# linomp/INF560-approximate-pattern-matching

Measured on AMD Instinct MI355X. Metric: window-DP-cells/sec, higher is better.
Workload: dtype u32

## Files before the change

inf560-approximate-pattern-matching_amd/csrc/apm_scan.hip:

```cpp
#include "apm_state.h"
#include "apm_core.h"

#include <algorithm>
#include <cstdlib>
#include <cstring>

__global__ void apm_popcount_kernel(const uint32_t *w, unsigned long long n, unsigned long long *sum) {
    unsigned long long acc = 0;
    for (unsigned long long i = (unsigned long long)blockIdx.x * blockDim.x + threadIdx.x; i < n; i += (unsigned long long)gridDim.x * blockDim.x)
        acc += (unsigned long long)__popc(w[i]);
    for (int d = 32; d; d >>= 1) acc += __shfl_down(acc, d, 64);
    if ((threadIdx.x & 63) == 0 && acc) atomicAdd(sum, acc);
}

__global__ void apm_popcount_listed_kernel(const uint32_t *w, const uint32_t *blist, const uint32_t *n_listed, const uint32_t *clist_cnt, int regions, unsigned long long *sum) {
    unsigned long long acc = 0;
    const unsigned long long n = (unsigned long long)*n_listed * 64ull, t0 = (unsigned long long)blockIdx.x * blockDim.x + threadIdx.x;
    for (unsigned long long i = t0; i < n; i += (unsigned long long)gridDim.x * blockDim.x)
        acc += (unsigned long long)__popc(w[(unsigned long long)blist[i >> 6] * 64ull + (i & 63ull)]);
    for (unsigned long long i = t0; i < (unsigned long long)regions; i += (unsigned long long)gridDim.x * blockDim.x) acc += clist_cnt[i];
    for (int d = 32; d; d >>= 1) acc += __shfl_down(acc, d, 64);
    if ((threadIdx.x & 63) == 0 && acc) atomicAdd(sum, acc);
}

// ... 163 lines not shown
    va.o_prefix = V.o_prefix;
    va.o_r2s = V.o_r2s;
    va.o_slots = V.o_slots;
    va.o_kext = V.o_kext;
    va.o_pat = V.o_pat;
    va.o_masks = V.o_masks;
    va.o_kinfo = V.o_kinfo;
    va.o_pinfo = V.o_pinfo;
    va.o_rc = V.o_rc;
    va.kinfo = D.d_kinfo;
    va.pinfo = reinterpret_cast<const uint2 *>(D.d_pinfo);
    va.kpart = D.d_kpart;
    va.pats = D.d_descs;
    va.n_pats = (int)V.descs.size();
    va.nk = (int)V.kinfo.size();
    va.band = g.band;
    va.code_shift = S.code_shift;
    va.stride = S.stride;
    return va;
}

static int run_fused(apm_ctx *ctx, DeviceState &ds, const ShardGeom &g, const SieveRange &r, ShortTails &tails, bool *ran) {
    const SievePlan &S = ctx->plan.sieve;
    bool fused_ok = scan_env().fused < 0 ? S.stride == 8 : scan_env().fused != 0;
    std::vector<ApmFusedArgs> fargs;
    std::vector<size_t> fa_index;
    for (size_t v = 0; fused_ok && v < S.launches.size(); ++v) {
        const VerifyLaunch &V = S.launches[v];
        DevVerify &D = ds.verify[v];
        ApmFusedArgs fa{};
        fa.s = sieve_args(S, g, r, ds.d_sieve_bmp);
        fa.v = verify_args(ctx, V, D, g, std::min<int64_t>(g.je, g.nrel - V.m_min + 1));
#ifdef APM_MEASURE
        if (!ds.d_stats) HIP_TRY(ctx, hipMalloc((void **)&ds.d_stats, APM_STATS_BYTES));
        fa.v.stats = ds.d_stats;
#endif
        if (!D.fused_threads) {
            D.fused_blocks_per_cu = apm_fused_geometry(fa, &D.fused_threads);
            if (D.fused_blocks_per_cu < 1) D.fused_threads = -1;
        }
        if (D.fused_threads < 64) fused_ok = false;
        if (fa.v.je > g.jb) { fargs.push_back(fa); fa_index.push_back(v); }
    }
    if (!fused_ok) return APM_OK;
    for (ApmFusedArgs &fa : fargs) {
        tails.ride_with(fa.s);
        const DevVerify &D = ds.verify[fa_index[&fa - fargs.data()]];
#ifdef APM_MEASURE
        HIP_TRY(ctx, hipMemsetAsync(ds.d_stats, 0, APM_STATS_BYTES, ds.stream));
#endif
        fa.v.work = ds.d_work;
        APM_LAUNCH(ctx, ds, "fused", APM_PICK(g, apm_launch_fused)(fa, D.fused_threads, ds.n_cu * D.fused_blocks_per_cu, &ds.work_epoch, ds.stream));
    }
    *ran = true;
    return APM_OK;
}

static int sieve_pass(apm_ctx *ctx, DeviceState &ds, const ShardGeom &g, SieveRange &r, ShortTails &tails, int v) {
    const SievePlan &S = ctx->plan.sieve;
    ApmSieve2Args sv = sieve_args(S, g, r, v < 0 ? ds.d_sieve_bmp : ds.verify[(size_t)v].d_bmp18);
    sv.masks = ds.d_masks;
    if (v >= 0) {
        const VerifyLaunch &V = S.launches[(size_t)v];
        const DevVerify &D = ds.verify[(size_t)v];
        sv.cf_image = reinterpret_cast<const uint4 *>(D.d_cf);
        sv.cf_len = (int)V.cf_image.size();
        sv.cf_o_rrec = V.cf_o_rrec;
// ... 1 lines not shown
        sv.cf_threads = D.cf_threads;
        sv.cf_blocks_per_cu = D.cf_blocks_per_cu;
        sv.cf_o_dp = V.cf_o_dp;
        sv.cf_dp_k = ctx->k;
        sv.cf_dp_cols = V.cf_dp_cols;
    }
    if (v < 0 || tails.n <= 512) tails.ride_with(sv);
    const bool use_blist = scan_env().blist && sv.cf_image != nullptr;
    r.blist_ctr = nullptr;
    if (use_blist) {
        sv.blist = ds.d_blist;
        sv.blist_ctr = APM_BLIST_CTR(ds.d_work, ds.sieve_epoch & 1);
        sv.blist_ctr_next = APM_BLIST_CTR(ds.d_work, (ds.sieve_epoch + 1) & 1);
        r.blist_ctr = sv.blist_ctr;
    }
    r.clist_regions = 0;
    if (use_blist && scan_env().clist) {
        const size_t want = (size_t)r.n_mask_blocks * (size_t)kClistPerBlock + (size_t)kClistMaxRegions * 64;
        const int grc = grow_device_buffer(ctx, ds, (void **)&ds.d_clist, &ds.clist_cap, want, 4);
        if (grc) return grc;
        if (!ds.d_clist_cnt) HIP_TRY(ctx, hipMalloc((void **)&ds.d_clist_cnt, (size_t)kClistMaxRegions * 4));
        const int regions = apm_sieve2cf_blocks(sv, ds.n_cu);
        if (regions >= 1 && regions <= kClistMaxRegions) {
            r.clist_regions = regions;
            r.clist_region_cap = scan_env().clist_region_cap ? (uint32_t)scan_env().clist_region_cap
                                                             : (uint32_t)std::max<int64_t>(64, r.n_mask_blocks * kClistPerBlock / regions);
            sv.clist = ds.d_clist;
            sv.clist_cnt = ds.d_clist_cnt;
            sv.clist_cap = r.clist_region_cap;
        }
    }
    ds.last_clist_regions = r.clist_regions;
    ds.last_blist_ctr = r.blist_ctr;
    HIP_TRY(ctx, APM_PICK(g, apm_launch_sieve2)(sv, ds.n_cu, ds.stream, scan_env().cf_dp_diag != 0, &ds.last_sieve_waves, &ds.last_cf_dp_form));
    if (use_blist) ++ds.sieve_epoch;
    return note_launch(ctx, ds, "sieve");
}

static int verify_pass(apm_ctx *ctx, DeviceState &ds, const ShardGeom &g, const SieveRange &r, size_t v, int64_t je_v) {
    DevVerify &D = ds.verify[v];
    ApmVerifyArgs va = verify_args(ctx, ctx->plan.sieve.launches[v], D, g, je_v);
    va.masks = ds.d_masks;
    if (r.blist_ctr) {
        va.blist = ds.d_blist;
        va.blist_ctr = r.blist_ctr;
    }
    if (r.clist_regions) {
        va.clist = ds.d_clist;
        va.clist_cnt = ds.d_clist_cnt;
        va.clist_cap = r.clist_region_cap;
        va.clist_regions = r.clist_regions;
        va.clist_min_batch = scan_env().clist_min_batch;
    }
    va.tile0 = r.p_lo;
    va.n_mask_blocks = r.n_mask_blocks;
#ifdef APM_MEASURE
    if (!ds.d_stats) HIP_TRY(ctx, hipMalloc((void **)&ds.d_stats, APM_STATS_BYTES));
    HIP_TRY(ctx, hipMemsetAsync(ds.d_stats, 0, APM_STATS_BYTES, ds.stream));
    va.stats = ds.d_stats;
#endif
    va.work = ds.d_work;
    if (!D.blocks_per_cu) D.blocks_per_cu = apm_verify_geometry(va, &D.threads);
    APM_LAUNCH(ctx, ds, "verify", APM_PICK(g, apm_launch_verify)(va, D.threads, ds.n_cu * D.blocks_per_cu, &ds.work_epoch, ds.stream));
    return APM_OK;
}

static int run_sieve_verify(apm_ctx *ctx, DeviceState &ds, const ShardGeom &g, SieveRange &r, ShortTails &tails) {
    const SievePlan &S = ctx->plan.sieve;
    r.n_mask_blocks = (r.nchunks() + 3) / 4;
    int rc = grow_device_buffer(ctx, ds, (void **)&ds.d_masks, &ds.masks_cap, (size_t)r.n_mask_blocks * 64 + 64, 4);
    if (rc) return rc;
    rc = grow_device_buffer(ctx, ds, (void **)&ds.d_blist, &ds.blist_cap, (size_t)r.n_mask_blocks + 64, 4);
    if (rc) return rc;
    ds.last_mask_blocks = r.n_mask_blocks;
    bool per_launch = S.per_launch_sieve;
    for (size_t v = 0; per_launch && v < S.launches.size(); ++v) {
        const VerifyLaunch &V = S.launches[v];
        DevVerify &D = ds.verify[v];
        if (!D.cf_threads) {
            D.cf_blocks_per_cu = apm_sieve2cf_geometry((int)V.cf_image.size(), apm_cf_dp_form(V.cf_o_dp > 0, ctx->k, scan_env().cf_dp_diag != 0), &D.cf_threads);
            if (D.cf_blocks_per_cu < 1) D.cf_threads = -1;
        }
        if (D.cf_threads < 64) per_launch = false;
    }
    bool any_pass = false;
    for (size_t v = 0; v < S.launches.size(); ++v) {
        const int64_t je_v = std::min<int64_t>(g.je, g.nrel - S.launches[v].m_min + 1);
        if (je_v <= g.jb) continue;
        if (per_launch || !any_pass) {
            rc = sieve_pass(ctx, ds, g, r, tails, per_launch ? (int)v : -1);
// ... 243 lines not shown
int scan_shard(apm_ctx *ctx, DeviceState &ds, const ShardText &sh, uint64_t own_begin, uint64_t own_end, unsigned long long *d_counts,
               const ApmPosSink *rec) {
    const uint8_t *d_text = sh.text;
    uint64_t text_off = sh.text_off, text_len = sh.text_len;
    const uint64_t n_total = sh.n_total;
    const bool sieve_on = ctx->plan.sieve.on;
    const uint64_t lim32 = (uint64_t)APM_SIEVE_MAX_BYTES - 4096;
    const uint64_t mis = (uint64_t)(reinterpret_cast<uintptr_t>(d_text) & 15u);
    if (sieve_on && mis != 0 && text_off >= mis && text_len > 0) {
        d_text -= mis;
        text_off -= mis;
        text_len += mis;
    }
    if (!sieve_on || text_len < lim32 || (reinterpret_cast<uintptr_t>(d_text) & 15u) != 0 || own_begin < text_off)
        return scan_shard_one(ctx, ds, ShardText{d_text, text_off, text_len, n_total}, own_begin, own_end, d_counts, rec);
    const uint64_t k = (uint64_t)ctx->k;
    const uint64_t oe = std::min(own_end, n_total > k ? n_total - k : 0);
    const uint64_t m_max = (uint64_t)std::max(ctx->plan.m_max, 1), step = (uint64_t)3 << 30;
    for (uint64_t b = own_begin; b < oe;) {
        const uint64_t e = std::min(oe, b + step);
        const uint64_t sb = text_off + ((b - text_off) & ~(uint64_t)15);
        const uint64_t se = std::min(text_off + text_len, e + m_max + 31);
        const int rc = scan_shard_one(ctx, ds, ShardText{d_text + (sb - text_off), sb, se - sb, n_total}, b, e, d_counts, rec);
        if (rc) return rc;
        b = e;
    }
    return APM_OK;
}

int sieve_candidates(apm_ctx *ctx, DeviceState &ds, double *value) {
    *value = 0;
    if (!ds.d_masks || ds.last_mask_blocks <= 0) return APM_OK;
    HIP_TRY(ctx, hipSetDevice(ds.dev));
    if (!ds.d_stats) HIP_TRY(ctx, hipMalloc((void **)&ds.d_stats, APM_STATS_BYTES));
    unsigned long long *d_sum = ds.d_stats + 7;
    HIP_TRY(ctx, hipMemsetAsync(d_sum, 0, 8, ds.stream));
    if (ds.last_clist_regions)
        hipLaunchKernelGGL(apm_popcount_listed_kernel, dim3(1024), dim3(256), 0, ds.stream, ds.d_masks, ds.d_blist, ds.last_blist_ctr, ds.d_clist_cnt, ds.last_clist_regions, d_sum);
    else
        hipLaunchKernelGGL(apm_popcount_kernel, dim3(1024), dim3(256), 0, ds.stream, ds.d_masks, (unsigned long long)ds.last_mask_blocks * 64ull, d_sum);
    unsigned long long h = 0;
    HIP_TRY(ctx, hipMemcpyAsync(&h, d_sum, 8, hipMemcpyDeviceToHost, ds.stream));
    HIP_TRY(ctx, hipStreamSynchronize(ds.stream));
    *value = (double)h;
    return APM_OK;
}
```

inf560-approximate-pattern-matching_amd/csrc/apm_sieve.h:

```cpp
#ifndef APM_SIEVE_H
#define APM_SIEVE_H

#include "apm_internal.h"

struct ApmSieve2Args {
    const uint8_t *text;
    int64_t avail_pad;
    int64_t tile0;
    int64_t nchunks;
    const uint4 *bitmap;
    int code_shift;
    int stride;
    uint32_t *masks;
    uint32_t *blist;
    uint32_t *blist_ctr, *blist_ctr_next;
    uint32_t *clist;
    uint32_t *clist_cnt;
    uint32_t clist_cap;
    int n_main_blocks;
    int n_tail;
    ApmTailArgs tail;
    const uint4 *cf_image;
    int cf_len, cf_o_rrec, cf_o_lrec;
    int cf_o_dp, cf_dp_k, cf_dp_cols;
    int cf_threads, cf_blocks_per_cu;
#ifdef APM_MEASURE
    int skip_mask;
#endif
};
#define APM_SIEVE_MAX_BYTES (((int64_t)1 << 32) - ((int64_t)64 << 20))
#define APM_CF_WAVE_BYTES 1552
#define APM_CF_DP_PEND_BYTES 128
#define APM_CF_DP_COLS 30
#define APM_CF_DP_SLOTS 7
static inline int apm_cf_dp_form(bool dp, int k, bool diag_on) { return !dp ? 0 : (diag_on && k <= 3 ? 2 : 1); }
const void *apm_sieve2cfdg_fn();
int apm_sieve2cf_geometry(int cf_len, int dp_form, int *threads);
int apm_sieve2cf_blocks(const ApmSieve2Args &a, int n_cu);

struct ApmVerifyArgs {
    const uint8_t *text;
    int64_t avail;
    int64_t avail_pad;
    int64_t jb, je, nrel;
    const uint4 *image;
    int image_len, o_prefix, o_r2s, o_slots, o_kext, o_pat;
    int o_masks;
    int o_rc;
    int o_kinfo, o_pinfo;
    const uint32_t *kinfo;
    const uint2 *pinfo;
    const uint32_t *kpart;
    const ApmPatDesc *pats;
    unsigned long long *counts;
    int n_pats, nk, k, band, code_shift;
    int stride;
    const uint32_t *masks;
    const uint32_t *blist;
    const uint32_t *blist_ctr;
    const uint32_t *clist;
    const uint32_t *clist_cnt;
    uint32_t clist_cap;
    int clist_regions;
    int clist_min_batch;
    int64_t tile0;
    int64_t n_mask_blocks;
    int n_blocks;
    uint32_t *work;
    int work_epoch;
    int work_groups;
#ifdef APM_MEASURE
    int skip_mask;
    unsigned long long *stats;
#endif
    ApmPosSink pos;
};

struct ApmFusedArgs {
    ApmSieve2Args s;
    ApmVerifyArgs v;
};
#define APM_FUSED_MAX_THREADS 896
hipError_t apm_launch_fused(const ApmFusedArgs &a, int threads, int max_blocks, int *work_epoch, hipStream_t s);
size_t apm_fused_lds_bytes(const ApmFusedArgs &a, int threads);
int apm_fused_geometry(const ApmFusedArgs &a, int *threads);

#define APM_WORK_GROUPS 32
#define APM_WORK_STRIDE 64
#define APM_WORK_BYTES (2 * APM_WORK_GROUPS * APM_WORK_STRIDE * 4 + 2 * APM_WORK_STRIDE * 4)
#define APM_BLIST_CTR(work, set) ((work) + 2 * APM_WORK_GROUPS * APM_WORK_STRIDE + (set) * APM_WORK_STRIDE)
#define APM_STATS_WAVES 16384
#define APM_STATS_BYTES (64 + 16 * APM_STATS_WAVES)
hipError_t apm_launch_sieve2(const ApmSieve2Args &a, int n_cu, hipStream_t s, bool dp_diag, int *cf_waves, int *cf_dp_form);
hipError_t apm_launch_verify(const ApmVerifyArgs &a, int threads, int max_blocks, int *work_epoch, hipStream_t s);
int apm_verify_geometry(const ApmVerifyArgs &a, int *threads);
#ifndef APM_REC
hipError_t apm_launch_fused_rec(const ApmFusedArgs &a, int threads, int max_blocks, int *work_epoch, hipStream_t s);
hipError_t apm_launch_sieve2_rec(const ApmSieve2Args &a, int n_cu, hipStream_t s, bool dp_diag, int *cf_waves, int *cf_dp_form);
hipError_t apm_launch_verify_rec(const ApmVerifyArgs &a, int threads, int max_blocks, int *work_epoch, hipStream_t s);
#endif

#endif
```

inf560-approximate-pattern-matching_amd/csrc/apm_sieve_body.h:

```cpp
#ifndef APM_SIEVE_BODY_H
#define APM_SIEVE_BODY_H
#include "apm_wave.h"
#include "apm_sieve.h"

#define APM_SIEVE2_BLOCK 512

template <bool CF, bool DP, bool DIAG = false>
__device__ __forceinline__ void apm_sieve2_body(const ApmSieve2Args &a, uint8_t *smem) {
    const int THREADS = CF ? (int)blockDim.x : APM_SIEVE2_BLOCK;
    constexpr uint32_t WAVE_BYTES = APM_CF_WAVE_BYTES + (DP ? APM_CF_DP_PEND_BYTES : 0);
    const int tid = threadIdx.x, lane = tid & 63;
    const int wv = __builtin_amdgcn_readfirstlane(tid >> 6);
    if ((int)blockIdx.x >= a.n_main_blocks) {
        apm_tail_body(a.tail, (int)blockIdx.x - a.n_main_blocks, reinterpret_cast<uint4 *>(smem), tid);
        return;
    }
    apm_stage_image(reinterpret_cast<uint4 *>(smem), a.bitmap, 2048, tid, THREADS);
    if constexpr (CF) apm_stage_image(reinterpret_cast<uint4 *>(smem + 32768), a.cf_image, a.cf_len >> 4, tid, THREADS);
    uint32_t *cl_ctr = reinterpret_cast<uint32_t *>(smem + 32768 + (CF ? a.cf_len + (THREADS / 64) * WAVE_BYTES : 0));
    if (CF && tid == 0) { cl_ctr[0] = 0u; cl_ctr[1] = DP ? 0u : 0xffffffffu; }
    __syncthreads();
    const int64_t W = (int64_t)a.n_main_blocks * (THREADS / 64);
    const int64_t nch = a.nchunks;

    const __amdgpu_buffer_rsrc_t rs_all =
        __builtin_amdgcn_make_buffer_rsrc(const_cast<uint8_t *>(a.text), 0, (int)(uint32_t)a.avail_pad, 0x00020000);
    const uint32_t t0_32 = (uint32_t)a.tile0, lane16 = 16u * (uint32_t)lane;
    auto load_chunk = [&](int64_t cc, u32x4 &r) __attribute__((always_inline)) {
        r = __builtin_amdgcn_raw_buffer_load_b128(rs_all, (int)(t0_32 + (uint32_t)cc * 1024u + lane16), 0, 0);
    };
    auto load_tail = [&](int64_t cc, v2u32 &tl) __attribute__((always_inline)) {
        tl = __builtin_amdgcn_raw_buffer_load_b64(rs_all, (int)(t0_32 + (uint32_t)cc * 1024u), 0, 0);
    };
    auto load_halo = [&](int64_t cc, u32x4 &hl) __attribute__((always_inline)) {
        const uint32_t g = (uint32_t)(a.tile0 + cc * 1024);
        const uint32_t off = lane < 2 ? g + 4096u + 16u * (uint32_t)lane : (lane == 2 ? g - 16u : 0xfffffff0u);
        hl = __builtin_amdgcn_raw_buffer_load_b128(rs_all, (int)off, 0, 0);
    };
    const uint32_t cs = (uint32_t)a.code_shift;
    auto pack16 = [&](const u32x4 &v) __attribute__((always_inline)) { return apm_pack16(v.x, v.y, v.z, v.w, cs); };
    auto hit_bits = [&](uint32_t slo, uint32_t nx0, int64_t cc) __attribute__((always_inline)) {
        uint32_t hits = apm_lookup2_chunk(slo, nx0);
#ifdef APM_MEASURE
        if (APM_SKIP(a, 1)) hits = 0;
#endif
        return cc < nch ? hits : 0u;
    };

    const uint2 *cf_tbl = reinterpret_cast<const uint2 *>(smem + 32768);
    const uint2 *cf_rrec = reinterpret_cast<const uint2 *>(smem + 32768 + a.cf_o_rrec);
    const uint2 *cf_lrec = reinterpret_cast<const uint2 *>(smem + 32768 + a.cf_o_lrec);
    uint32_t *st = reinterpret_cast<uint32_t *>(smem + 32768 + a.cf_len + wv * WAVE_BYTES);
    uint32_t *mk = st + 260;
    uint16_t *rq = reinterpret_cast<uint16_t *>(mk + 64);
    uint16_t *pend = rq + 128;
    const uint4 *cf_dp = reinterpret_cast<const uint4 *>(smem + 32768 + a.cf_o_dp);
    uint32_t qe = 0, qlo = 0, qhi = 0, qn = 0;
    auto dp_flush = [&]() __attribute__((always_inline)) {
        const bool valid = (uint32_t)lane < qn && qe != 0xffffffffu;
        bool keep = false;
#ifdef APM_MEASURE
        if (APM_SKIP(a, 4)) keep = valid;
        else
#endif
        if (valid) {
            const uint4 tb = cf_dp[(qhi >> 28) & 7u];
            if constexpr (DIAG) {
                uint32_t t0, t1;
                apm_code_planes(qlo, qhi & 0x0fffffffu, t0, t1);
                keep = a.cf_dp_k >= 2 ? apm_code_dp_diag<1>(tb.x, tb.y, (int)(tb.z & 0xffu), t0, t1, a.cf_dp_k)
                                      : apm_code_dp_diag<0>(tb.x, tb.y, (int)(tb.z & 0xffu), t0, t1, a.cf_dp_k);
            } else {
                const uint32_t cw[2] = {qlo, qhi};
                keep = apm_code_dp_pass<2>(tb.x, tb.y, (int)(tb.z & 0xffu), cw, a.cf_dp_cols, a.cf_dp_k);
            }
        }
#ifdef APM_MEASURE
        if (APM_SKIP(a, 2)) keep = valid;
#endif
        for (unsigned long long sm = __builtin_amdgcn_ballot_w64(keep); sm;) {
            const int l = __builtin_ctzll(sm);
            const uint32_t el = (uint32_t)__builtin_amdgcn_readlane((int)qe, l);
            if (keep && qe == el && lane != l) keep = false;
            sm = __builtin_amdgcn_ballot_w64(keep) & ~((2ull << l) - 1ull);
        }
        const unsigned long long km = __builtin_amdgcn_ballot_w64(keep);
        const uint32_t nk = (uint32_t)__builtin_popcountll(km);
        uint32_t base = 0;
        if (lane == 0) {
            if (qn > nk) __hip_atomic_fetch_sub(&cl_ctr[1], qn - nk, __ATOMIC_RELAXED, __HIP_MEMORY_SCOPE_WORKGROUP);
            if (nk) base = __hip_atomic_fetch_add(&cl_ctr[0], nk, __ATOMIC_RELAXED, __HIP_MEMORY_SCOPE_WORKGROUP);
        }
        base = (uint32_t)__builtin_amdgcn_readfirstlane((int)base);
        if (keep) a.clist[(size_t)blockIdx.x * a.clist_cap + base + apm_wave_rank(km)] = qe;
        qn = 0;
    };
    auto cf_filter = [&](uint32_t hm, const uint32_t (&sc)[4], uint32_t hc, uint32_t e0) __attribute__((always_inline)) -> uint32_t {
        if (!__builtin_amdgcn_ballot_w64(hm != 0u)) return 0u;
#pragma unroll
        for (int j = 0; j < 4; ++j) st[1 + 64 * j + lane] = sc[j];
        if (lane < 4) st[lane < 2 ? 257 + lane : (lane == 2 ? 0 : 259)] = hc;
        mk[lane] = 0u;
        uint32_t qh = 0, qt = 0;
        uint32_t pn = 0;
        auto run_batch = [&](uint32_t nb) __attribute__((always_inline)) {
            const bool split = nb <= 32u;
            const uint32_t ei = split ? ((uint32_t)lane & 31u) : (uint32_t)lane;
            const uint32_t ent = rq[(qh + ei) & 127u];
            const bool valid = ei < nb;
            const bool take0 = !split || lane < 32, take1 = !split || lane >= 32;
            const uint32_t se = 2u * (ent & 2047u), d = 1u + (se >> 4), she = 2u * (se & 15u);
            const uint32_t w0 = st[d], w1 = st[d + 1u];
            const uint32_t x0 = __builtin_amdgcn_alignbit(w1, w0, she) & 0xffffu, x1 = __builtin_amdgcn_alignbit(w1, w0, she + 2u) & 0xffffu;
            const uint2 t0 = cf_tbl[x0 & 2047u], t1 = cf_tbl[x1 & 2047u];
            const bool p0 = valid && take0 && !(ent & 2048u) && ((t0.x >> (x0 >> 11)) & 1u), p1 = valid && take1 && ((t1.x >> (x1 >> 11)) & 1u);
            const unsigned long long both = __builtin_amdgcn_ballot_w64(p0 && p1);
            if (both) {
                const uint32_t idx = qt + apm_wave_rank(both);
                if (p0 && p1) rq[idx & 127u] = (uint16_t)(ent | 2048u);
                qt += (uint32_t)__builtin_popcountll(both);
            }
            bool act = p0 || p1;
            const uint32_t s = se + (p0 ? 0u : 1u);
            const uint32_t c0 = __builtin_amdgcn_alignbit(w1, w0, she + (p0 ? 0u : 2u));
            const uint32_t x = p0 ? x0 : x1, word = p0 ? t0.x : t1.x, pre = p0 ? t0.y : t1.y, bit = x >> 11;
            uint2 rec = cf_rrec[act ? pre + (uint32_t)__builtin_popcount(word & ((1u << bit) - 1u)) : 0u];
            uint32_t li = 0;
            bool in_list = false;
            if ((rec.x >> 30) == 3u) { li = rec.x & 0xffffu; in_list = true; rec = cf_lrec[li]; ++li; }
            while (__builtin_amdgcn_ballot_w64(act)) {
                const uint32_t side = rec.x >> 30;
                const uint32_t uu = side == 2u ? s : s + 16u + ((rec.y >> 20) & 0xffu);
                const bool vis = uu <= 4128u;
                const uint32_t ua = vis ? uu : 16u;
                uint32_t tw = __builtin_amdgcn_alignbit(st[(ua >> 4) + 1u], st[ua >> 4], 2u * (ua & 15u));
                if (side == 2u) tw = apm_rev_codes(tw);
                const bool ok = apm_cf_pass(rec.x, rec.y, c0, tw, vis);
                bool pass = act && ok;
                if constexpr (DP) {
                    const uint32_t slot = (rec.y >> 28) & 7u;
                    const bool want = pass && slot != 0u;
                    const unsigned long long wm = __builtin_amdgcn_ballot_w64(want);
                    if (wm) {
                        const uint32_t idx = pn + apm_wave_rank(wm);
                        if (want && idx < 64u) { pend[idx] = (uint16_t)(s | (slot << 13)); pass = false; }
                        pn += (uint32_t)__builtin_popcountll(wm);
                        pn = pn < 64u ? pn : 64u;
                    }
                }
                if (pass) {
                    atomicOr(&mk[(s >> 4) & 63u], 1u << (8u * (s >> 10) + ((s & 15u) >> 1)));
                    act = false;
                } else if (act) {
                    if (!in_list || (rec.y >> 31)) act = false;
                    else { rec = cf_lrec[li]; ++li; }
                }
            }
        };
        {
            const uint32_t cnt = (uint32_t)__builtin_popcount(hm);
            const uint32_t inc = apm_wave_incl_scan(cnt);
            const uint32_t total = (uint32_t)__builtin_amdgcn_readlane((int)inc, 63);
            if (total <= 128u) {
                uint32_t pos = inc - cnt;
                while (__builtin_amdgcn_ballot_w64(hm != 0u)) {
                    if (hm != 0u) {
                        const uint32_t t = (uint32_t)__builtin_ctz(hm);
                        hm &= hm - 1u;
                        rq[pos & 127u] = (uint16_t)(512u * (t >> 3) + 8u * (uint32_t)lane + (t & 7u));
                        ++pos;
                    }
                }
                qt = total;
                while (qt - qh >= 64u) { run_batch(64u); qh += 64u; }
            }
        }
        while (__builtin_amdgcn_ballot_w64(hm != 0u)) {
            const bool has = hm != 0u;
            const uint32_t t = has ? (uint32_t)__builtin_ctz(hm) : 0u;
            hm &= hm - 1u;
            apm_wave_append(rq, qt, has, 512u * (t >> 3) + 8u * (uint32_t)lane + (t & 7u), 127u);
            while (qt - qh >= 64u) { run_batch(64u); qh += 64u; }
        }
        while (qt != qh) { const uint32_t nb = qt - qh < 64u ? qt - qh : 64u; run_batch(nb); qh += nb; }
        if constexpr (DP) {
            if (pn) {
                if (qn + pn > 64u) dp_flush();
                uint32_t room = 0;
                if (lane == 0) room = __hip_atomic_fetch_add(&cl_ctr[1], pn, __ATOMIC_RELAXED, __HIP_MEMORY_SCOPE_WORKGROUP) + pn <= a.clist_cap;
                const uint32_t pi = (uint32_t)lane - qn;
                const bool mine = pi < pn;
                const uint32_t ent = pend[mine ? pi : 0u];
                const uint32_t s = ent & 8191u, slot = ent >> 13;
                const uint32_t info = cf_dp[slot].z;
                const int rk = DIAG ? a.cf_dp_k >> 1 : a.cf_dp_k;
                const int r = (int)s - (int)((info >> 8) & 0xffu) - rk;
                const int rlen = DIAG ? (int)(info & 0xffu) + 2 * rk : (int)(info >> 16);
                const bool inside = r >= -16 && r + rlen <= 4128;
                const uint32_t u = (uint32_t)(r + 16), d = inside ? u >> 4 : 0u, sh = 2u * (u & 15u);
                const uint32_t w0 = st[d], w1 = st[d + 1u], w2 = st[d + 2u];
                const uint32_t lo = __builtin_amdgcn_alignbit(w1, w0, sh);
                const uint32_t hi = (__builtin_amdgcn_alignbit(w2, w1, sh) & 0x0fffffffu) | (slot << 28);
                room = (uint32_t)__builtin_amdgcn_readfirstlane((int)room);
                if (!room && lane == 0) __hip_atomic_fetch_sub(&cl_ctr[1], pn, __ATOMIC_RELAXED, __HIP_MEMORY_SCOPE_WORKGROUP);
                uint32_t *mw = &mk[(s >> 4) & 63u];
                const uint32_t mbit = 1u << (8u * (s >> 10) + ((s & 15u) >> 1));
                if (mine && !(room && inside)) atomicOr(mw, mbit);
                if (room) {
                    const bool drop = (*mw & mbit) != 0u;
                    if (mine) {
                        qe = drop ? 0xffffffffu : e0 + (s >> 1);
                        qlo = lo;
                        qhi = hi;
                    }
                    qn += pn;
                }
            }
        }
        return mk[lane];
    };

    uint32_t bl_pend = 0, bl_n = 0;
    auto bl_flush = [&]() __attribute__((always_inline)) {
        uint32_t base = 0;
        if (lane == 0) base = __hip_atomic_fetch_add(a.blist_ctr, bl_n, __ATOMIC_RELAXED, __HIP_MEMORY_SCOPE_AGENT);
        base = (uint32_t)__builtin_amdgcn_readfirstlane((int)base);
        if ((uint32_t)lane < bl_n) a.blist[base + (uint32_t)lane] = bl_pend;
        bl_n = 0;
    };
    if (CF && a.blist && blockIdx.x == 0 && tid == 0) *a.blist_ctr_next = 0u;

    int64_t c = ((int64_t)blockIdx.x * (THREADS / 64) + wv) * 4;
    u32x4 r0, r1, r2, r3, hl;
    v2u32 tl;
    load_chunk(c, r0);
    load_chunk(c + 1, r1);
    load_chunk(c + 2, r2);
    load_chunk(c + 3, r3);
    if constexpr (CF) load_halo(c, hl);
    else load_tail(c + 4, tl);
    for (; c < nch; c += 4 * W) {
        const uint32_t s0 = pack16(r0), s1 = pack16(r1), s2 = pack16(r2), s3 = pack16(r3);
        uint32_t s4;
        if constexpr (CF) s4 = pack16(hl);
        else s4 = apm_pack4(tl.x, cs) | (apm_pack4(tl.y, cs) << 8);
        load_chunk(c + 4 * W, r0);
        load_chunk(c + 4 * W + 1, r1);
        load_chunk(c + 4 * W + 2, r2);
        load_chunk(c + 4 * W + 3, r3);
        if constexpr (CF) load_halo(c + 4 * W, hl);
        else load_tail(c + 4 * W + 4, tl);
        const uint32_t h0 = hit_bits(s0, (uint32_t)__builtin_amdgcn_readfirstlane((int)s1), c);
        __builtin_amdgcn_sched_barrier(0);
        const uint32_t h1 = hit_bits(s1, (uint32_t)__builtin_amdgcn_readfirstlane((int)s2), c + 1);
        __builtin_amdgcn_sched_barrier(0);
        const uint32_t h2 = hit_bits(s2, (uint32_t)__builtin_amdgcn_readfirstlane((int)s3), c + 2);
        __builtin_amdgcn_sched_barrier(0);
        const uint32_t h3 = hit_bits(s3, (uint32_t)__builtin_amdgcn_readfirstlane((int)s4), c + 3);
        uint32_t hm = (h0 >> 24) | ((h1 >> 24) << 8) | ((h2 >> 24) << 16) | (h3 & 0xff000000u);
        if constexpr (CF) {
            const uint32_t e0b = (uint32_t)((a.tile0 + (c >> 2) * 4096) >> 1);
            __builtin_amdgcn_sched_barrier(0);
            const uint32_t sc[4] = {s0, s1, s2, s3};
            hm = cf_filter(hm, sc, s4, e0b);
        }
        if constexpr (CF) {
            if (a.clist) {
                const uint32_t e0 = (uint32_t)((a.tile0 + (c >> 2) * 4096) >> 1) + 8u * (uint32_t)lane;
                uint32_t *region = a.clist + (size_t)blockIdx.x * a.clist_cap;
                for (;;) {
                    const bool has = hm != 0u;
                    const unsigned long long mask = __builtin_amdgcn_ballot_w64(has);
                    if (!mask) break;
                    const uint32_t n = (uint32_t)__builtin_popcountll(mask);
                    uint32_t base = 0;
                    if constexpr (DP) {
                        uint32_t fits = 0;
                        if (lane == 0) {
                            const uint32_t old = __hip_atomic_fetch_add(&cl_ctr[1], n, __ATOMIC_RELAXED, __HIP_MEMORY_SCOPE_WORKGROUP);
                            fits = old + n <= a.clist_cap;
                            if (fits) base = __hip_atomic_fetch_add(&cl_ctr[0], n, __ATOMIC_RELAXED, __HIP_MEMORY_SCOPE_WORKGROUP);
                            else __hip_atomic_fetch_sub(&cl_ctr[1], n, __ATOMIC_RELAXED, __HIP_MEMORY_SCOPE_WORKGROUP);
                        }
                        base = (uint32_t)__builtin_amdgcn_readfirstlane((int)base);
                        if (!__builtin_amdgcn_readfirstlane((int)fits)) break;
                    } else {
                        if (lane == 0) base = __hip_atomic_fetch_add(&cl_ctr[0], n, __ATOMIC_RELAXED, __HIP_MEMORY_SCOPE_WORKGROUP);
                        base = (uint32_t)__builtin_amdgcn_readfirstlane((int)base);
                        if (base + n > a.clist_cap) {
                            if (lane == 0) __hip_atomic_fetch_min(&cl_ctr[1], base, __ATOMIC_RELAXED, __HIP_MEMORY_SCOPE_WORKGROUP);
                            break;
                        }
                    }
                    const uint32_t t = has ? (uint32_t)__builtin_ctz(hm) : 0u;
                    hm &= hm - 1u;
                    if (has)
                        region[base + apm_wave_rank(mask)] = e0 + 512u * (t >> 3) + (t & 7u);
                }
            }
            const bool any = __builtin_amdgcn_ballot_w64(hm != 0u) != 0ull;
            if (!a.clist || any) a.masks[(size_t)(c >> 2) * 64 + (size_t)lane] = hm;
            if (a.blist && any) {
                if ((uint32_t)lane == bl_n) bl_pend = (uint32_t)(c >> 2);
                if (++bl_n == 64u) bl_flush();
            }
        } else {
            a.masks[(size_t)(c >> 2) * 64 + (size_t)lane] = hm;
        }
    }
    if (DP && qn) dp_flush();
    if constexpr (CF) {
        if (a.blist) {
            if ((uint32_t)lane < bl_n) st[lane] = bl_pend;
            if (lane == 0) st[64] = bl_n;
            __syncthreads();
            uint32_t *wg = reinterpret_cast<uint32_t *>(smem + 32768 + a.cf_len);
            const uint32_t nw = (uint32_t)(THREADS / 64);
            uint32_t before = 0, total = 0;
            for (uint32_t w = 0; w < nw; ++w) {
                const uint32_t cw = wg[w * (WAVE_BYTES / 4) + 64];
                if (w < (uint32_t)wv) before += cw;
                total += cw;
            }
            uint32_t *gbase = wg + 65;
            if (tid == 0 && total) *gbase = __hip_atomic_fetch_add(a.blist_ctr, total, __ATOMIC_RELAXED, __HIP_MEMORY_SCOPE_AGENT);
            __syncthreads();
            if ((uint32_t)lane < bl_n) a.blist[*gbase + before + (uint32_t)lane] = bl_pend;
            if (a.clist && tid == 0) a.clist_cnt[blockIdx.x] = DP ? cl_ctr[0] : (cl_ctr[0] < cl_ctr[1] ? cl_ctr[0] : cl_ctr[1]);
        }
    }
}

#endif
```

inf560-approximate-pattern-matching_amd/csrc/apm_stats.hip:

```cpp
#include "apm_runtime.h"
#include "apm_core.h"

#include <cstdlib>
#include <string>
#include <vector>

void account(apm_ctx *ctx, uint64_t n_total, uint64_t ob, uint64_t oe) {
    const uint64_t k = (uint64_t)ctx->k;
    const uint64_t limit = n_total > k ? n_total - k : 0;
    oe = std::min(oe, limit);
    if (oe <= ob) return;
    for (const auto &p : ctx->pats) {
        const uint64_t m = (uint64_t)p.m;
        const uint64_t full_end = n_total >= m ? std::min<uint64_t>(oe, n_total - m + 1) : 0;
        const uint64_t nfull = full_end > ob ? full_end - ob : 0;
        double cells = double(nfull) * double(m) * double(m);
        for (uint64_t j = std::max(ob, full_end); j < oe; ++j) {
            const double s = double(n_total - j);
            cells += s * s;
        }
        ctx->timing.windows += oe - ob;
        ctx->timing.cells_algorithmic += cells;
        if (p.kernel == APM_KERNEL_BANDED || p.kernel == APM_KERNEL_NFA)
            ctx->timing.cells_evaluated += double(oe - ob) * double(m) * double(2 * (ctx->k / 2) + 1);
// ... 127 lines not shown
            HIP_TRY(ctx, hipEventSynchronize(ds.ev_sq[at + 1]));
            float t = 0;
            HIP_TRY(ctx, hipEventElapsedTime(&t, ds.ev_sq[at], ds.ev_sq[at + 1]));
            *value = t;
        }
        return APM_OK;
    }
    if (n == "occ_segment") { *value = (double)ds.occ_segment; return APM_OK; }
    if (n == "occ_lanes") { *value = (double)ds.occ_lanes; return APM_OK; }
    if (n == "best_ms") {
        *value = 0.0;
        if (ds.best_timed) {
            HIP_TRY(ctx, hipSetDevice(ds.dev));
            HIP_TRY(ctx, hipEventSynchronize(ds.ev_best[1]));
            float t = 0;
            HIP_TRY(ctx, hipEventElapsedTime(&t, ds.ev_best[0], ds.ev_best[1]));
            *value = t;
        }
        return APM_OK;
    }
    if (n == "norm_ms" || n == "map_ms") {
        const int at = n == "norm_ms" ? 0 : 2;
        *value = 0.0;
        if (at == 0 ? ds.tn_timed : ds.map_timed) {
            HIP_TRY(ctx, hipSetDevice(ds.dev));
            HIP_TRY(ctx, hipEventSynchronize(ds.ev_tn[at + 1]));
            float t = 0;
            HIP_TRY(ctx, hipEventElapsedTime(&t, ds.ev_tn[at], ds.ev_tn[at + 1]));
            *value = t;
        }
        return APM_OK;
    }
#ifdef APM_MEASURE
    if (n.rfind("verify_", 0) == 0 && ds.d_stats) {
        HIP_TRY(ctx, hipSetDevice(ds.dev));
        HIP_TRY(ctx, hipStreamSynchronize(ds.stream));
        unsigned long long h[8] = {};
        HIP_TRY(ctx, hipMemcpy(h, ds.d_stats, 64, hipMemcpyDeviceToHost));
        if (n == "verify_survivors") { *value = (double)h[1]; return APM_OK; }
        if (n == "verify_dp_items") { *value = (double)h[2]; return APM_OK; }
        if (n == "verify_counted") { *value = (double)h[3]; return APM_OK; }
        if (n.rfind("verify_wave_", 0) == 0) {
            std::vector<unsigned long long> t(2 * APM_STATS_WAVES);
            HIP_TRY(ctx, hipMemcpy(t.data(), ds.d_stats + 8, t.size() * 8, hipMemcpyDeviceToHost));
            std::vector<double> st, en;
            unsigned long long t0 = ~0ull;
            for (size_t w = 0; w < APM_STATS_WAVES; ++w) if (t[2 * w + 1]) t0 = std::min(t0, t[2 * w]);
            for (size_t w = 0; w < APM_STATS_WAVES; ++w) if (t[2 * w + 1]) { st.push_back((double)(t[2 * w] - t0) * 0.01); en.push_back((double)(t[2 * w + 1] - t0) * 0.01); }
            if (n.rfind("verify_wave_grp", 0) == 0 || n.rfind("verify_wave_xcd", 0) == 0) {
                const bool by_xcd = n[12] == 'x';
                const int want = atoi(n.c_str() + 18);
                double lo = 1e30, hi = 0, sum = 0; long cnt = 0;
                for (size_t w = 0; w < APM_STATS_WAVES; ++w) {
                    if (!t[2 * w + 1]) continue;
                    const int key = by_xcd ? (int)((w / 4) % 8) : (int)((w ^ (w >> 5)) % APM_WORK_GROUPS);
                    if (key != want) continue;
                    const double e = (double)(t[2 * w + 1] - t0) * 0.01;
                    lo = std::min(lo, e); hi = std::max(hi, e); sum += e; ++cnt;
                }
                *value = n[15] == 'm' && n[16] == 'a' ? hi : (n[15] == 'm' && n[16] == 'i' ? lo : (cnt ? sum / cnt : 0));
                return APM_OK;
            }
            if (n.rfind("verify_wave_slow", 0) == 0) {
                const bool end = n.rfind("verify_wave_slowend", 0) == 0;
                const size_t want = (size_t)atoi(n.c_str() + (end ? 19 : 16));
                std::vector<std::pair<unsigned long long, size_t>> by_end;
// ... 24 lines not shown
```

inf560-approximate-pattern-matching_amd/csrc/apm_wave.h:

```cpp
#ifndef APM_WAVE_H
#define APM_WAVE_H

#include "apm_device.h"

typedef unsigned int v2u32 __attribute__((ext_vector_type(2)));
typedef __attribute__((address_space(3))) uint32_t apm_lds_u32;

__device__ __forceinline__ uint32_t apm_udot4(uint32_t a, uint32_t b) {
    return __builtin_amdgcn_udot4(a, b, 0u, false);
}

__device__ __forceinline__ uint32_t apm_pack16(uint32_t x, uint32_t y, uint32_t z, uint32_t w, uint32_t cs) {
    const uint32_t mask = 0x03030303u << cs;
    const uint32_t p0 = apm_udot4(x & mask, 0x40100401u), p1 = apm_udot4(y & mask, 0x40100401u);
    const uint32_t p2 = apm_udot4(z & mask, 0x40100401u), p3 = apm_udot4(w & mask, 0x40100401u);
    return (p0 >> cs) | (p1 << (8u - cs)) | (p2 << (16u - cs)) | (p3 << (24u - cs));
}

__device__ __forceinline__ uint32_t apm_pack4(uint32_t w, uint32_t cs) {
    return apm_udot4((w >> cs) & 0x03030303u, 0x40100401u);
}

__device__ __forceinline__ uint32_t apm_wave_rank(unsigned long long mask) {
    return __builtin_amdgcn_mbcnt_hi((uint32_t)(mask >> 32), __builtin_amdgcn_mbcnt_lo((uint32_t)mask, 0u));
}

template <typename T>
__device__ __forceinline__ void apm_wave_append(T *dst, uint32_t &count, bool has, uint32_t value, uint32_t wrap = 0xffffffffu) {
    const unsigned long long mask = __builtin_amdgcn_ballot_w64(has);
    if (has) dst[(count + apm_wave_rank(mask)) & wrap] = (T)value;
    count += (uint32_t)__builtin_popcountll(mask);
}

__device__ __forceinline__ uint32_t apm_wave_incl_scan(uint32_t v) {
    v += (uint32_t)__builtin_amdgcn_update_dpp(0, (int)v, 0x111, 0xf, 0xf, false);
    v += (uint32_t)__builtin_amdgcn_update_dpp(0, (int)v, 0x112, 0xf, 0xf, false);
    v += (uint32_t)__builtin_amdgcn_update_dpp(0, (int)v, 0x114, 0xf, 0xf, false);
    v += (uint32_t)__builtin_amdgcn_update_dpp(0, (int)v, 0x118, 0xf, 0xf, false);
    v += (uint32_t)__builtin_amdgcn_update_dpp(0, (int)v, 0x142, 0xa, 0xf, false);
    v += (uint32_t)__builtin_amdgcn_update_dpp(0, (int)v, 0x143, 0xc, 0xf, false);
    return v;
}

__device__ __forceinline__ uint32_t apm_lookup2_chunk(uint32_t slo, uint32_t nx0) {
    const uint32_t shi = (uint32_t)__builtin_amdgcn_update_dpp((int)nx0, (int)slo, 0x130, 0xf, 0xf, false);
    uint32_t hits = 0;
#pragma unroll
    for (int t = 0; t < 8; ++t) {
        const uint32_t y = t ? __builtin_amdgcn_alignbit(shi, slo, 4u * (uint32_t)t - 2u) : (slo << 2);
        const uint32_t word = *(const apm_lds_u32 *)(uintptr_t)(y & 0x7ffcu);
        hits = __builtin_amdgcn_alignbit(word >> ((y >> 15) & 31u), hits, 1u);
    }
    return hits;
}

struct ApmKeyList {
    const uint32_t *s_bmp;
    const uint16_t *s_prefix, *s_r2s, *s_slots;
    __device__ __forceinline__ uint32_t first(uint32_t x) const {
        const uint32_t bit = x >> 11, word = s_bmp[x & 2047u];
        const uint32_t e = s_r2s[(uint32_t)s_prefix[x & 2047u] + (uint32_t)__builtin_popcount(word & ((1u << bit) - 1u))];
        return (e & 0x8000u) ? e : ((uint32_t)s_slots[e] | ((e + 1u) << 16));
    }
    __device__ __forceinline__ uint32_t next(uint32_t cur) const { return (uint32_t)s_slots[cur >> 16] | ((cur & 0xffff0000u) + 0x10000u); }
// ... 7 lines not shown
```

Measured before the change: 785300000 billion.

## Streamline DIAG sieve batch path and add measure-only census counters

In the DIAG variant of the sieve body, the split batch now has each half-wave evaluate its own offset directly, which drops the paired ballot and requeue step. The change also moves the LDS room-reservation atomic after the DP loads, swaps the workgroup atomics for inline single-lane ds_add/ds_sub asm, and removes the wraparound mask and upper-bound check in DIAG mode. It further adds per-wave census counters and a stats query, compiled only under APM_MEASURE. The aim is fewer instructions and less atomic latency on the candidate-filter path, at some risk of correctness assumptions about queue bounds in DIAG mode.

```diff
diff --git a/inf560-approximate-pattern-matching_amd/csrc/apm_scan.hip b/inf560-approximate-pattern-matching_amd/csrc/apm_scan.hip
--- a/inf560-approximate-pattern-matching_amd/csrc/apm_scan.hip
+++ b/inf560-approximate-pattern-matching_amd/csrc/apm_scan.hip
@@ -219,7 +219,7 @@
         fa.s = sieve_args(S, g, r, ds.d_sieve_bmp);
         fa.v = verify_args(ctx, V, D, g, std::min<int64_t>(g.je, g.nrel - V.m_min + 1));
 #ifdef APM_MEASURE
-        if (!ds.d_stats) HIP_TRY(ctx, hipMalloc((void **)&ds.d_stats, APM_STATS_BYTES));
+        if (!ds.d_stats) HIP_TRY(ctx, hipMalloc((void **)&ds.d_stats, APM_STATS_ALLOC));
         fa.v.stats = ds.d_stats;
 #endif
         if (!D.fused_threads) {
@@ -287,6 +287,11 @@
     }
     ds.last_clist_regions = r.clist_regions;
     ds.last_blist_ctr = r.blist_ctr;
+#ifdef APM_MEASURE
+    if (!ds.d_stats) HIP_TRY(ctx, hipMalloc((void **)&ds.d_stats, APM_STATS_ALLOC));
+    sv.census = ds.d_stats + APM_CENSUS_AT;
+    HIP_TRY(ctx, hipMemsetAsync(sv.census, 0, APM_CENSUS_N * 8, ds.stream));
+#endif
     HIP_TRY(ctx, APM_PICK(g, apm_launch_sieve2)(sv, ds.n_cu, ds.stream, scan_env().cf_dp_diag != 0, &ds.last_sieve_waves, &ds.last_cf_dp_form));
     if (use_blist) ++ds.sieve_epoch;
     return note_launch(ctx, ds, "sieve");
@@ -310,7 +315,7 @@
     va.tile0 = r.p_lo;
     va.n_mask_blocks = r.n_mask_blocks;
 #ifdef APM_MEASURE
-    if (!ds.d_stats) HIP_TRY(ctx, hipMalloc((void **)&ds.d_stats, APM_STATS_BYTES));
+    if (!ds.d_stats) HIP_TRY(ctx, hipMalloc((void **)&ds.d_stats, APM_STATS_ALLOC));
     HIP_TRY(ctx, hipMemsetAsync(ds.d_stats, 0, APM_STATS_BYTES, ds.stream));
     va.stats = ds.d_stats;
 #endif
@@ -620,7 +625,7 @@
     *value = 0;
     if (!ds.d_masks || ds.last_mask_blocks <= 0) return APM_OK;
     HIP_TRY(ctx, hipSetDevice(ds.dev));
-    if (!ds.d_stats) HIP_TRY(ctx, hipMalloc((void **)&ds.d_stats, APM_STATS_BYTES));
+    if (!ds.d_stats) HIP_TRY(ctx, hipMalloc((void **)&ds.d_stats, APM_STATS_ALLOC));
     unsigned long long *d_sum = ds.d_stats + 7;
     HIP_TRY(ctx, hipMemsetAsync(d_sum, 0, 8, ds.stream));
     if (ds.last_clist_regions)
diff --git a/inf560-approximate-pattern-matching_amd/csrc/apm_sieve.h b/inf560-approximate-pattern-matching_amd/csrc/apm_sieve.h
--- a/inf560-approximate-pattern-matching_amd/csrc/apm_sieve.h
+++ b/inf560-approximate-pattern-matching_amd/csrc/apm_sieve.h
@@ -26,8 +26,10 @@
     int cf_threads, cf_blocks_per_cu;
 #ifdef APM_MEASURE
     int skip_mask;
+    unsigned long long *census;
 #endif
 };
+#define APM_CENSUS_N 16
 #define APM_SIEVE_MAX_BYTES (((int64_t)1 << 32) - ((int64_t)64 << 20))
 #define APM_CF_WAVE_BYTES 1552
 #define APM_CF_DP_PEND_BYTES 128
@@ -91,6 +93,12 @@
 #define APM_BLIST_CTR(work, set) ((work) + 2 * APM_WORK_GROUPS * APM_WORK_STRIDE + (set) * APM_WORK_STRIDE)
 #define APM_STATS_WAVES 16384
 #define APM_STATS_BYTES (64 + 16 * APM_STATS_WAVES)
+#ifdef APM_MEASURE
+#define APM_CENSUS_AT (APM_STATS_BYTES / 8)
+#define APM_STATS_ALLOC (APM_STATS_BYTES + 8 * APM_CENSUS_N)
+#else
+#define APM_STATS_ALLOC APM_STATS_BYTES
+#endif
 hipError_t apm_launch_sieve2(const ApmSieve2Args &a, int n_cu, hipStream_t s, bool dp_diag, int *cf_waves, int *cf_dp_form);
 hipError_t apm_launch_verify(const ApmVerifyArgs &a, int threads, int max_blocks, int *work_epoch, hipStream_t s);
 int apm_verify_geometry(const ApmVerifyArgs &a, int *threads);
diff --git a/inf560-approximate-pattern-matching_amd/csrc/apm_sieve_body.h b/inf560-approximate-pattern-matching_amd/csrc/apm_sieve_body.h
--- a/inf560-approximate-pattern-matching_amd/csrc/apm_sieve_body.h
+++ b/inf560-approximate-pattern-matching_amd/csrc/apm_sieve_body.h
@@ -4,6 +4,11 @@
 #include "apm_sieve.h"
 
 #define APM_SIEVE2_BLOCK 512
+#ifdef APM_MEASURE
+#define APM_CENSUS(i, n) (cz[i] += (uint32_t)(n))
+#else
+#define APM_CENSUS(i, n) ((void)0)
+#endif
 
 template <bool CF, bool DP, bool DIAG = false>
 __device__ __forceinline__ void apm_sieve2_body(const ApmSieve2Args &a, uint8_t *smem) {
@@ -22,6 +27,9 @@
     __syncthreads();
     const int64_t W = (int64_t)a.n_main_blocks * (THREADS / 64);
     const int64_t nch = a.nchunks;
+#ifdef APM_MEASURE
+    uint32_t cz[11] = {};
+#endif
 
     const __amdgpu_buffer_rsrc_t rs_all =
         __builtin_amdgcn_make_buffer_rsrc(const_cast<uint8_t *>(a.text), 0, (int)(uint32_t)a.avail_pad, 0x00020000);
@@ -56,7 +64,17 @@
     uint16_t *pend = rq + 128;
     const uint4 *cf_dp = reinterpret_cast<const uint4 *>(smem + 32768 + a.cf_o_dp);
     uint32_t qe = 0, qlo = 0, qhi = 0, qn = 0;
+    auto cl_add = [&](int i, uint32_t v) __attribute__((always_inline)) -> uint32_t {
+        if constexpr (DIAG) return apm_lds_add_rtn_1lane(&cl_ctr[i], v);
+        else return __hip_atomic_fetch_add(&cl_ctr[i], v, __ATOMIC_RELAXED, __HIP_MEMORY_SCOPE_WORKGROUP);
+    };
+    auto cl_sub = [&](int i, uint32_t v) __attribute__((always_inline)) {
+        if constexpr (DIAG) apm_lds_sub_1lane(&cl_ctr[i], v);
+        else __hip_atomic_fetch_sub(&cl_ctr[i], v, __ATOMIC_RELAXED, __HIP_MEMORY_SCOPE_WORKGROUP);
+    };
     auto dp_flush = [&]() __attribute__((always_inline)) {
+        APM_CENSUS(7, 1);
+        APM_CENSUS(8, qn);
         const bool valid = (uint32_t)lane < qn && qe != 0xffffffffu;
         bool keep = false;
 #ifdef APM_MEASURE
@@ -88,8 +106,8 @@
         const uint32_t nk = (uint32_t)__builtin_popcountll(km);
         uint32_t base = 0;
         if (lane == 0) {
-            if (qn > nk) __hip_atomic_fetch_sub(&cl_ctr[1], qn - nk, __ATOMIC_RELAXED, __HIP_MEMORY_SCOPE_WORKGROUP);
-            if (nk) base = __hip_atomic_fetch_add(&cl_ctr[0], nk, __ATOMIC_RELAXED, __HIP_MEMORY_SCOPE_WORKGROUP);
+            if (qn > nk) cl_sub(1, qn - nk);
+            if (nk) base = cl_add(0, nk);
         }
         base = (uint32_t)__builtin_amdgcn_readfirstlane((int)base);
         if (keep) a.clist[(size_t)blockIdx.x * a.clist_cap + base + apm_wave_rank(km)] = qe;
@@ -97,6 +115,7 @@
     };
     auto cf_filter = [&](uint32_t hm, const uint32_t (&sc)[4], uint32_t hc, uint32_t e0) __attribute__((always_inline)) -> uint32_t {
         if (!__builtin_amdgcn_ballot_w64(hm != 0u)) return 0u;
+        APM_CENSUS(1, 1);
 #pragma unroll
         for (int j = 0; j < 4; ++j) st[1 + 64 * j + lane] = sc[j];
         if (lane < 4) st[lane < 2 ? 257 + lane : (lane == 2 ? 0 : 259)] = hc;
@@ -104,31 +123,53 @@
         uint32_t qh = 0, qt = 0;
         uint32_t pn = 0;
         auto run_batch = [&](uint32_t nb) __attribute__((always_inline)) {
-            const bool split = nb <= 32u;
-            const uint32_t ei = split ? ((uint32_t)lane & 31u) : (uint32_t)lane;
-            const uint32_t ent = rq[(qh + ei) & 127u];
-            const bool valid = ei < nb;
-            const bool take0 = !split || lane < 32, take1 = !split || lane >= 32;
-            const uint32_t se = 2u * (ent & 2047u), d = 1u + (se >> 4), she = 2u * (se & 15u);
-            const uint32_t w0 = st[d], w1 = st[d + 1u];
-            const uint32_t x0 = __builtin_amdgcn_alignbit(w1, w0, she) & 0xffffu, x1 = __builtin_amdgcn_alignbit(w1, w0, she + 2u) & 0xffffu;
-            const uint2 t0 = cf_tbl[x0 & 2047u], t1 = cf_tbl[x1 & 2047u];
-            const bool p0 = valid && take0 && !(ent & 2048u) && ((t0.x >> (x0 >> 11)) & 1u), p1 = valid && take1 && ((t1.x >> (x1 >> 11)) & 1u);
-            const unsigned long long both = __builtin_amdgcn_ballot_w64(p0 && p1);
-            if (both) {
-                const uint32_t idx = qt + apm_wave_rank(both);
-                if (p0 && p1) rq[idx & 127u] = (uint16_t)(ent | 2048u);
-                qt += (uint32_t)__builtin_popcountll(both);
-            }
-            bool act = p0 || p1;
-            const uint32_t s = se + (p0 ? 0u : 1u);
-            const uint32_t c0 = __builtin_amdgcn_alignbit(w1, w0, she + (p0 ? 0u : 2u));
-            const uint32_t x = p0 ? x0 : x1, word = p0 ? t0.x : t1.x, pre = p0 ? t0.y : t1.y, bit = x >> 11;
+            bool act;
+            uint32_t s, c0, x, word, pre;
+            if (DIAG && nb <= 32u) {
+                APM_CENSUS(3, 1);
+                const uint32_t odd = (uint32_t)lane >> 5, ei = (uint32_t)lane & 31u;
+                const uint32_t ent = rq[(qh + ei) & 127u];
+                const uint32_t se = 2u * (ent & 2047u), d = 1u + (se >> 4);
+                s = se + odd;
+                c0 = __builtin_amdgcn_alignbit(st[d + 1u], st[d], 2u * (s & 15u));
+                x = c0 & 0xffffu;
+                const uint2 t = cf_tbl[x & 2047u];
+                word = t.x;
+                pre = t.y;
+                act = ei < nb && (ent & 2048u) <= (odd << 11) && ((word >> (x >> 11)) & 1u);
+            } else {
+                const bool split = nb <= 32u;
+                if (split) APM_CENSUS(3, 1);
+                else APM_CENSUS(4, 1);
+                const uint32_t ei = split ? ((uint32_t)lane & 31u) : (uint32_t)lane;
+                const uint32_t ent = rq[(qh + ei) & 127u];
+                const bool valid = ei < nb;
+                const bool take0 = !split || lane < 32, take1 = !split || lane >= 32;
+                const uint32_t se = 2u * (ent & 2047u), d = 1u + (se >> 4), she = 2u * (se & 15u);
+                const uint32_t w0 = st[d], w1 = st[d + 1u];
+                const uint32_t x0 = __builtin_amdgcn_alignbit(w1, w0, she) & 0xffffu, x1 = __builtin_amdgcn_alignbit(w1, w0, she + 2u) & 0xffffu;
+                const uint2 t0 = cf_tbl[x0 & 2047u], t1 = cf_tbl[x1 & 2047u];
+                const bool p0 = valid && take0 && !(ent & 2048u) && ((t0.x >> (x0 >> 11)) & 1u), p1 = valid && take1 && ((t1.x >> (x1 >> 11)) & 1u);
+                const unsigned long long both = __builtin_amdgcn_ballot_w64(p0 && p1);
+                if (both) {
+                    const uint32_t idx = qt + apm_wave_rank(both);
+                    if (p0 && p1) rq[idx & 127u] = (uint16_t)(ent | 2048u);
+                    qt += (uint32_t)__builtin_popcountll(both);
+                }
+                act = p0 || p1;
+                s = se + (p0 ? 0u : 1u);
+                c0 = __builtin_amdgcn_alignbit(w1, w0, she + (p0 ? 0u : 2u));
+                x = p0 ? x0 : x1;
+                word = p0 ? t0.x : t1.x;
+                pre = p0 ? t0.y : t1.y;
+            }
+            const uint32_t bit = x >> 11;
             uint2 rec = cf_rrec[act ? pre + (uint32_t)__builtin_popcount(word & ((1u << bit) - 1u)) : 0u];
             uint32_t li = 0;
             bool in_list = false;
             if ((rec.x >> 30) == 3u) { li = rec.x & 0xffffu; in_list = true; rec = cf_lrec[li]; ++li; }
             while (__builtin_amdgcn_ballot_w64(act)) {
+                APM_CENSUS(5, 1);
                 const uint32_t side = rec.x >> 30;
                 const uint32_t uu = side == 2u ? s : s + 16u + ((rec.y >> 20) & 0xffu);
                 const bool vis = uu <= 4128u;
@@ -164,10 +205,11 @@
             if (total <= 128u) {
                 uint32_t pos = inc - cnt;
                 while (__builtin_amdgcn_ballot_w64(hm != 0u)) {
+                    APM_CENSUS(2, 1);
                     if (hm != 0u) {
                         const uint32_t t = (uint32_t)__builtin_ctz(hm);
                         hm &= hm - 1u;
-                        rq[pos & 127u] = (uint16_t)(512u * (t >> 3) + 8u * (uint32_t)lane + (t & 7u));
+                        rq[DIAG ? pos : (pos & 127u)] = (uint16_t)(512u * (t >> 3) + 8u * (uint32_t)lane + (t & 7u));
                         ++pos;
                     }
                 }
@@ -176,6 +218,7 @@
             }
         }
         while (__builtin_amdgcn_ballot_w64(hm != 0u)) {
+            APM_CENSUS(2, 1);
             const bool has = hm != 0u;
             const uint32_t t = has ? (uint32_t)__builtin_ctz(hm) : 0u;
             hm &= hm - 1u;
@@ -185,9 +228,10 @@
         while (qt != qh) { const uint32_t nb = qt - qh < 64u ? qt - qh : 64u; run_batch(nb); qh += nb; }
         if constexpr (DP) {
             if (pn) {
+                APM_CENSUS(6, 1);
                 if (qn + pn > 64u) dp_flush();
                 uint32_t room = 0;
-                if (lane == 0) room = __hip_atomic_fetch_add(&cl_ctr[1], pn, __ATOMIC_RELAXED, __HIP_MEMORY_SCOPE_WORKGROUP) + pn <= a.clist_cap;
+                if constexpr (!DIAG) { if (lane == 0) room = cl_add(1, pn) + pn <= a.clist_cap; }
                 const uint32_t pi = (uint32_t)lane - qn;
                 const bool mine = pi < pn;
                 const uint32_t ent = pend[mine ? pi : 0u];
@@ -196,13 +240,14 @@
                 const int rk = DIAG ? a.cf_dp_k >> 1 : a.cf_dp_k;
                 const int r = (int)s - (int)((info >> 8) & 0xffu) - rk;
                 const int rlen = DIAG ? (int)(info & 0xffu) + 2 * rk : (int)(info >> 16);
-                const bool inside = r >= -16 && r + rlen <= 4128;
+                const bool inside = r >= -16 && (DIAG || r + rlen <= 4128);
                 const uint32_t u = (uint32_t)(r + 16), d = inside ? u >> 4 : 0u, sh = 2u * (u & 15u);
                 const uint32_t w0 = st[d], w1 = st[d + 1u], w2 = st[d + 2u];
                 const uint32_t lo = __builtin_amdgcn_alignbit(w1, w0, sh);
                 const uint32_t hi = (__builtin_amdgcn_alignbit(w2, w1, sh) & 0x0fffffffu) | (slot << 28);
+                if constexpr (DIAG) { if (lane == 0) room = cl_add(1, pn) + pn <= a.clist_cap; }
                 room = (uint32_t)__builtin_amdgcn_readfirstlane((int)room);
-                if (!room && lane == 0) __hip_atomic_fetch_sub(&cl_ctr[1], pn, __ATOMIC_RELAXED, __HIP_MEMORY_SCOPE_WORKGROUP);
+                if (!room && lane == 0) cl_sub(1, pn);
                 uint32_t *mw = &mk[(s >> 4) & 63u];
                 const uint32_t mbit = 1u << (8u * (s >> 10) + ((s & 15u) >> 1));
                 if (mine && !(room && inside)) atomicOr(mw, mbit);
@@ -240,6 +285,7 @@
     if constexpr (CF) load_halo(c, hl);
     else load_tail(c + 4, tl);
     for (; c < nch; c += 4 * W) {
+        APM_CENSUS(0, 1);
         const uint32_t s0 = pack16(r0), s1 = pack16(r1), s2 = pack16(r2), s3 = pack16(r3);
         uint32_t s4;
         if constexpr (CF) s4 = pack16(hl);
@@ -272,6 +318,7 @@
                     const bool has = hm != 0u;
                     const unsigned long long mask = __builtin_amdgcn_ballot_w64(has);
                     if (!mask) break;
+                    APM_CENSUS(9, 1);
                     const uint32_t n = (uint32_t)__builtin_popcountll(mask);
                     uint32_t base = 0;
                     if constexpr (DP) {
@@ -308,7 +355,15 @@
             a.masks[(size_t)(c >> 2) * 64 + (size_t)lane] = hm;
         }
     }
-    if (DP && qn) dp_flush();
+    if (DP && qn) {
+        APM_CENSUS(10, 1);
+        dp_flush();
+    }
+#ifdef APM_MEASURE
+    if (a.census && lane == 0)
+        for (int i = 0; i < 11; ++i)
+            if (cz[i]) atomicAdd(&a.census[i], (unsigned long long)cz[i]);
+#endif
     if constexpr (CF) {
         if (a.blist) {
             if ((uint32_t)lane < bl_n) st[lane] = bl_pend;
diff --git a/inf560-approximate-pattern-matching_amd/csrc/apm_stats.hip b/inf560-approximate-pattern-matching_amd/csrc/apm_stats.hip
--- a/inf560-approximate-pattern-matching_amd/csrc/apm_stats.hip
+++ b/inf560-approximate-pattern-matching_amd/csrc/apm_stats.hip
@@ -183,6 +183,16 @@
         return APM_OK;
     }
 #ifdef APM_MEASURE
+    if (n.rfind("sieve_census_", 0) == 0 && ds.d_stats) {
+        const int i = atoi(n.c_str() + 13);
+        if (i < 0 || i >= APM_CENSUS_N) return APM_ERR_INVALID;
+        HIP_TRY(ctx, hipSetDevice(ds.dev));
+        HIP_TRY(ctx, hipStreamSynchronize(ds.stream));
+        unsigned long long c = 0;
+        HIP_TRY(ctx, hipMemcpy(&c, ds.d_stats + APM_CENSUS_AT + i, 8, hipMemcpyDeviceToHost));
+        *value = (double)c;
+        return APM_OK;
+    }
     if (n.rfind("verify_", 0) == 0 && ds.d_stats) {
         HIP_TRY(ctx, hipSetDevice(ds.dev));
         HIP_TRY(ctx, hipStreamSynchronize(ds.stream));
diff --git a/inf560-approximate-pattern-matching_amd/csrc/apm_wave.h b/inf560-approximate-pattern-matching_amd/csrc/apm_wave.h
--- a/inf560-approximate-pattern-matching_amd/csrc/apm_wave.h
+++ b/inf560-approximate-pattern-matching_amd/csrc/apm_wave.h
@@ -30,6 +30,15 @@
     const unsigned long long mask = __builtin_amdgcn_ballot_w64(has);
     if (has) dst[(count + apm_wave_rank(mask)) & wrap] = (T)value;
     count += (uint32_t)__builtin_popcountll(mask);
+}
+
+__device__ __forceinline__ uint32_t apm_lds_add_rtn_1lane(const uint32_t *p, uint32_t v) {
+    uint32_t old;
+    asm volatile("ds_add_rtn_u32 %0, %1, %2\n\ts_waitcnt lgkmcnt(0)" : "=&v"(old) : "v"((uint32_t)(uintptr_t)(const apm_lds_u32 *)p), "v"(v) : "memory");
+    return old;
+}
+__device__ __forceinline__ void apm_lds_sub_1lane(const uint32_t *p, uint32_t v) {
+    asm volatile("ds_sub_u32 %0, %1" : : "v"((uint32_t)(uintptr_t)(const apm_lds_u32 *)p), "v"(v) : "memory");
 }
 
 __device__ __forceinline__ uint32_t apm_wave_incl_scan(uint32_t v) {
```

Result: faster. 813300000 billion, median of 6 (+3.6%).
